# HKUST-Aerial-Robotics/DenseSurfelMapping

Measured on NVIDIA B200. Metric: frames/sec (KITTI 1226x370 depth+gray), higher is better.
Workload: dtype f32

## Files before the change

densesurfelmapping_b200/csrc/dsm_tile.cu:

```cuda
#include "dsm_exact.cuh"
#include <cuda_pipeline.h>

__device__ __forceinline__ unsigned smem_u32(const void *p) { return (unsigned)__cvta_generic_to_shared(p); }
__device__ __forceinline__ void mbar_init(unsigned bar, unsigned count)
{
    asm volatile("mbarrier.init.shared::cta.b64 [%0], %1;" ::"r"(bar), "r"(count) : "memory");
    asm volatile("fence.mbarrier_init.release.cluster;" ::: "memory");
}
__device__ __forceinline__ void mbar_expect_tx(unsigned bar, unsigned bytes)
{
    asm volatile("mbarrier.arrive.expect_tx.shared::cta.b64 _, [%0], %1;" ::"r"(bar), "r"(bytes) : "memory");
}
__device__ __forceinline__ void mbar_wait(unsigned bar, unsigned parity)
{
    unsigned ok = 0;
    for (unsigned spin = 0; !ok; spin++)
    {
        asm volatile("{\n\t.reg .pred p;\n\tmbarrier.try_wait.parity.shared::cta.b64 p, [%1], %2;\n\tselp.u32 %0, 1, 0, p;\n\t}"
                     : "=r"(ok)
                     : "r"(bar), "r"(parity)
                     : "memory");
        if (!ok && spin > (1u << 20)) __trap();
    }
}
__device__ __forceinline__ void tma_load_3d(unsigned dst, const CUtensorMap *map, int x, int y, int z, unsigned bar)
{
    asm volatile("cp.async.bulk.tensor.3d.shared::cluster.global.mbarrier::complete_tx::bytes [%0], [%1, {%3, %4, %5}], [%2];" ::"r"(dst),
                 "l"(reinterpret_cast<unsigned long long>(map)), "r"(bar), "r"(x), "r"(y), "r"(z)
                 : "memory");
}

#define A_EPS 3.814697265625e-06f
#define A_ALPHA 1e-10f
#define A_BIG 1e30f

__device__ __forceinline__ void relax_frame(const DsmDev &d, int b, int tid, int nthreads)
{
    const int n = __ldcg(&d.nlist[b]);
    if (n > 0)
    {
        const size_t fo = (size_t)b * d.px_stride;
        int2 *list = d.list + fo;
        int32_t *labels = d.labels + fo;
        uint8_t *codes = d.code + fo;
        int32_t *t = d.tstable + (size_t)b * d.S;
        for (;;)
        {
            int changed = 0;
            for (int e = tid; e < n; e += nthreads)
            {
                const int2 en = __ldcg(&list[e]);
                if (en.x < 0) continue;
                const int owner = __ldcg(&labels[en.x]);
                if (__ldcg(&t[owner]) < en.x)
                {
                    const int win = en.y & 0x0fffffff;
                    labels[en.x] = win;
                    codes[en.x] = (uint8_t)(en.y >> 28);
                    list[e].x = -1;
                    if (__ldcg(&t[win]) > en.x) atomicMin(&t[win], en.x);
                    changed = 1;
                }
            }
            if (!__syncthreads_or(changed)) break;
        }
    }
    if (tid == 0)
    {
        d.nlist[b] = 0;
        d.done[b] = 0;
    }
}

__device__ __forceinline__ float pick4(float a0, float a1, float a2, float a3, int i)
{
    return i == 0 ? a0 : (i == 1 ? a1 : (i == 2 ? a2 : a3));
}

#define DSM_CODE_NONE 4

template <bool FIRST>
__global__ void __launch_bounds__(128, 8) k_assign2(const __grid_constant__ DsmDev d)
{
    pdl_enter();
    __shared__ int s_last;
    const int b = d.frame0 + blockIdx.z;
    const int x4 = (blockIdx.x * 64 + threadIdx.x) * 4;
    const int y = blockIdx.y * blockDim.y + threadIdx.y;
    const int lane = threadIdx.x & 31;
    const bool active = (x4 < d.W) && (y < d.H);

    const size_t fo = (size_t)b * d.px_stride;
    const size_t so = (size_t)b * d.S;
    int wc[4] = {DSM_CODE_NONE, DSM_CODE_NONE, DSM_CODE_NONE, DSM_CODE_NONE};
    int oc[4] = {0, 0, 0, 0};
    int sidx0 = 0;
    if (active)
    {
        const size_t po = fo + (size_t)y * d.Wp + x4;
        const uchar4 g4 = *reinterpret_cast<const uchar4 *>(d.gray + po);
        float iv[4];
        if (FIRST)
        {
            const float4 z4 = *reinterpret_cast<const float4 *>(d.depth + po);
            iv[0] = (z4.x > F_0p01_LO) ? __frcp_rn(z4.x) : 0.0f;
            iv[1] = (z4.y > F_0p01_LO) ? __frcp_rn(z4.y) : 0.0f;
            iv[2] = (z4.z > F_0p01_LO) ? __frcp_rn(z4.z) : 0.0f;
            iv[3] = (z4.w > F_0p01_LO) ? __frcp_rn(z4.w) : 0.0f;
            *reinterpret_cast<float4 *>(d.invd + po) = make_float4(iv[0], iv[1], iv[2], iv[3]);
        }
        else
        {
            const float4 i4 = *reinterpret_cast<const float4 *>(d.invd + po);
            iv[0] = i4.x, iv[1] = i4.y, iv[2] = i4.z, iv[3] = i4.w;
            const uchar4 c4 = *reinterpret_cast<const uchar4 *>(d.code + po);
            oc[0] = c4.x, oc[1] = c4.y, oc[2] = c4.z, oc[3] = c4.w;
        }
        const float gi[4] = {(float)g4.x, (float)g4.y, (float)g4.z, (float)g4.w};
        const int bx = x4 >> 3, by = y >> 3, rx0 = x4 & 7, ry = y & 7;
        const int xa = (rx0 == 0) ? bx - 1 : bx, xb = xa + 1;
        const int ya = (ry < 4) ? by - 1 : by, yb = ya + 1;
        const bool vxa = xa >= 0 && xa < d.spw, vxb = xb >= 0 && xb < d.spw;
        const bool vya = ya >= 0 && ya < d.sph, vyb = (ry != 4) && yb >= 0 && yb < d.sph;
        sidx0 = ya * d.spw + xa;
        float sxq[4], sxq0[4], ayy[4], sI[4], shi[4], slo[4];
        bool sv[4];
        bool allmd = true, allmd0 = true;
        const float fyq = (float)y * 0.25f;
#pragma unroll
        for (int c = 0; c < 4; c++)
        {
            sv[c] = ((c >> 1) ? vxb : vxa) && ((c & 1) ? vyb : vya);
            const int li = sv[c] ? sidx0 + (c & 1) * d.spw + (c >> 1) : 0;
            const float4 s4 = d.seed[so + li];
            const float2 hl = d.seed_hl[so + li];
            sxq[c] = sv[c] ? s4.x * 0.25f : 1e18f;
            sxq0[c] = ((c >> 1) && rx0 == 4) ? 1e18f : sxq[c];
            const float ay = s4.y * 0.25f - fyq;
            ayy[c] = ay * ay;
            sI[c] = s4.z, shi[c] = hl.x, slo[c] = hl.y;
            const bool mdpos = s4.w > 0.f || !sv[c];
            allmd &= mdpos;
            if (!(c >> 1)) allmd0 &= mdpos;
        }
        if (rx0 != 4) allmd0 = allmd;
        unsigned uncertain = 0;
#pragma unroll
        for (int i = 0; i < 4; i++)
        {
            const float fxq = (float)(x4 + i) * 0.25f;
            const float pi = gi[i], pv = iv[i];
            const float w = (pv > 0.f && (i == 0 ? allmd0 : allmd)) ? 400.f : 0.f;
            float cost[4];
#pragma unroll
            for (int c = 0; c < 4; c++)
            {
                const float ax = (i == 0 ? sxq0[c] : sxq[c]) - fxq;
                const float n = fmaf(ax, ax, ayy[c]);
                const float idf = sI[c] - pi;
                const float cn = fmaf(idf * idf, 0.01f, n);
                const float t = (shi[c] - pv) + slo[c];
                cost[c] = fmaf(t * t, w, cn);
            }
            const float lo01 = fminf(cost[0], cost[1]), hi01 = fmaxf(cost[0], cost[1]);
            const float lo23 = fminf(cost[2], cost[3]), hi23 = fmaxf(cost[2], cost[3]);
            const float m1 = fminf(lo01, lo23);
            const float m2 = fminf(fminf(fmaxf(lo01, lo23), fminf(hi01, hi23)), A_BIG);
            wc[i] = cost[0] == m1 ? 0 : (cost[1] == m1 ? 1 : (cost[2] == m1 ? 2 : 3));
            const bool certain = (m2 - m1 > A_EPS * (m2 + m1) + A_ALPHA) && (m1 < 9e5f);
            if (!certain) uncertain |= 1u << i;
        }
        if (uncertain)
        {
            SeedC sc[4];
#pragma unroll
            for (int c = 0; c < 4; c++)
            {
                const int li = sv[c] ? sidx0 + (c & 1) * d.spw + (c >> 1) : 0;
                const float4 s4 = d.seed[so + li];
                sc[c].x = s4.x, sc[c].y = s4.y, sc[c].I = s4.z, sc[c].md = s4.w;
                sc[c].inv = d.inv_md[so + li];
            }
            const float fy = (float)y;
            while (uncertain)
            {
                const int i = __ffs(uncertain) - 1;
                uncertain &= uncertain - 1;
                const float fx = (float)(x4 + i);
                const float my_i = pick4(gi[0], gi[1], gi[2], gi[3], i);
                const float my_inv = pick4(iv[0], iv[1], iv[2], iv[3], i);
                const double my_inv_d = (double)my_inv;
                float min_d = 1e6f, min_nd = 1e6f;
                int idx_d = DSM_CODE_NONE, idx_nd = DSM_CODE_NONE;
                bool all_has_depth = true;
#pragma unroll
                for (int c = 0; c < 4; c++)
                {
                    const bool valid = sv[c] && ((c >> 1) ? !(rx0 == 4 && i == 0) : true);
                    float cnd, cdd;
                    const bool has = calc_cost(sc[c], my_i, my_inv, my_inv_d, fx, fy, cnd, cdd);
                    cdd = valid ? cdd : __int_as_float(0x7f800000);
                    cnd = valid ? cnd : __int_as_float(0x7f800000);
                    all_has_depth &= has || !valid;
                    const bool bd = cdd < min_d, bn = cnd < min_nd;
                    min_d = bd ? cdd : min_d;
                    idx_d = bd ? c : idx_d;
                    min_nd = bn ? cnd : min_nd;
                    idx_nd = bn ? c : idx_nd;
                }
                const int wv = all_has_depth ? idx_d : idx_nd;
                wc[0] = i == 0 ? wv : wc[0];
                wc[1] = i == 1 ? wv : wc[1];
                wc[2] = i == 2 ? wv : wc[2];
                wc[3] = i == 3 ? wv : wc[3];
            }
        }
#pragma unroll
        for (int i = 0; i < 4; i++)
            if (x4 + i >= d.W) wc[i] = DSM_CODE_NONE;
    }
    const int spw = d.spw;
    auto seed_of = [&](int c) { return c == DSM_CODE_NONE ? 0 : sidx0 + (c & 1) * spw + (c >> 1); };

    if (FIRST)
    {
        if (active)
        {
            const size_t po = fo + (size_t)y * d.Wp + x4;
            *reinterpret_cast<int4 *>(d.labels + po) = make_int4(seed_of(wc[0]), seed_of(wc[1]), seed_of(wc[2]), seed_of(wc[3]));
            *reinterpret_cast<uchar4 *>(d.code + po) = make_uchar4(wc[0], wc[1], wc[2], wc[3]);
        }
        return;
    }

    int2 ent[4];
    int nent = 0;
    if (active)
    {
        bool changed = false;
        const int32_t *ts = d.tstable + so;
#pragma unroll
        for (int i = 0; i < 4; i++)
        {
            if (x4 + i >= d.W || wc[i] == DSM_CODE_NONE || wc[i] == oc[i]) continue;
            const int pidx = y * d.Wp + x4 + i;
            const int win = seed_of(wc[i]);
            if (ts[seed_of(oc[i])] < 0)
            {
                oc[i] = wc[i];
                changed = true;
                if (ts[win] > pidx) atomicMin(&d.tstable[so + win], pidx);
            }
            else
            {
                ent[nent++] = make_int2(pidx, win | (wc[i] << 28));
            }
        }
        if (changed)
        {
            const size_t po = fo + (size_t)y * d.Wp + x4;
            *reinterpret_cast<int4 *>(d.labels + po) = make_int4(seed_of(oc[0]), seed_of(oc[1]), seed_of(oc[2]), seed_of(oc[3]));
            *reinterpret_cast<uchar4 *>(d.code + po) = make_uchar4(oc[0], oc[1], oc[2], oc[3]);
        }
    }
    if (__any_sync(FULL, nent > 0))
    {
        int total;
        const int excl = warp_excl_scan(nent, lane, total);
        int base = 0;
        if (lane == 31) base = atomicAdd(&d.nlist[b], total);
        base = __shfl_sync(FULL, base, 31);
        int2 *list = d.list + fo;
        for (int j = 0; j < nent; j++) list[base + excl + j] = ent[j];
    }
    const int tid = threadIdx.y * 64 + threadIdx.x;
    __syncthreads();
    if (tid == 0)
    {
        __threadfence();
        s_last = (atomicAdd(&d.done[b], 1) == (int)(gridDim.x * gridDim.y) - 1) ? 1 : 0;
    }
    __syncthreads();
    if (s_last)
    {
        __threadfence();
        relax_frame(d, b, tid, 128);
    }
}

#define DL_STRIDE 232
#define TILE_PLANE_BYTES 12544
#define TILE_BYTE_PLANE 4608
#define GAT_SMEM_DEP 0
#define GAT_SMEM_COD TILE_PLANE_BYTES
#define GAT_SMEM_GRY (TILE_PLANE_BYTES + TILE_BYTE_PLANE)
#define GAT_SMEM_LIST (TILE_PLANE_BYTES + 2 * TILE_BYTE_PLANE)
#define GAT_SMEM_ND (GAT_SMEM_LIST + 16 * DL_STRIDE * 4)
#define GAT_SMEM_BAR (GAT_SMEM_ND + 16 * 4)
#define GAT_SMEM_BYTES (GAT_SMEM_BAR + 16)
#define TILE_TX_BYTES (DSM_TILE_W * DSM_TILE_H * 4u + 2u * DSM_TILE_GW * DSM_TILE_H)

__device__ __forceinline__ unsigned zero_bytes_to_nibble(unsigned x)
{
    unsigned t = (x & 0x7f7f7f7fu) + 0x7f7f7f7fu;
    t = ~(t | x | 0x7f7f7f7fu);
    return ((t >> 7) * 0x00204081u >> 21) & 0xfu;
}
__device__ __forceinline__ unsigned member_mask16(const unsigned *codes, int r)
{
    const unsigned lo = (r < 8) ? 0x01010101u : 0u;
    const unsigned e_left = 0x02020202u | lo, e_right = lo;
    return zero_bytes_to_nibble(codes[0] ^ e_left) | (zero_bytes_to_nibble(codes[1] ^ e_left) << 4) |
           (zero_bytes_to_nibble(codes[2] ^ e_right) << 8) | (zero_bytes_to_nibble(codes[3] ^ e_right) << 12);
}

__device__ __forceinline__ int mask_index_sum(unsigned m)
{
    return __popc(m & 0xaaaau) + 2 * __popc(m & 0xccccu) + 4 * __popc(m & 0xf0f0u) + 8 * __popc(m & 0xff00u);
}
__device__ __forceinline__ unsigned nibble_to_bytes(unsigned n) { return (((n & 0xfu) * 0x00204081u) & 0x01010101u) * 0xffu; }

__global__ void __launch_bounds__(256, 6) k_gather(const __grid_constant__ DsmDev d, const __grid_constant__ DsmMaps mp)
{
    pdl_enter();
    extern __shared__ __align__(128) unsigned char smem[];
    const float *t_dep = reinterpret_cast<const float *>(smem + GAT_SMEM_DEP);
    const uint8_t *t_cod = smem + GAT_SMEM_COD, *t_gry = smem + GAT_SMEM_GRY;
    float *lists = reinterpret_cast<float *>(smem + GAT_SMEM_LIST);
    int *s_nd = reinterpret_cast<int *>(smem + GAT_SMEM_ND);
    const unsigned bar = smem_u32(smem + GAT_SMEM_BAR);

    const int b = d.frame0 + blockIdx.z;
    const int warp = threadIdx.x >> 5, lane = threadIdx.x & 31;
    const int X0 = blockIdx.x * (DSM_TILE_SX * DSM_SP) - DSM_SP / 2, Y0 = blockIdx.y * (DSM_TILE_SY * DSM_SP) - DSM_SP / 2;
    if (threadIdx.x == 0)
    {
        mbar_init(bar, 1);
        mbar_expect_tx(bar, TILE_TX_BYTES);
        tma_load_3d(smem_u32(smem + GAT_SMEM_DEP), &mp.dep, X0, Y0, b, bar);
        tma_load_3d(smem_u32(smem + GAT_SMEM_COD), &mp.cod, X0 - DSM_TILE_GX, Y0, b, bar);
        tma_load_3d(smem_u32(smem + GAT_SMEM_GRY), &mp.gry, X0 - DSM_TILE_GX, Y0, b, bar);
    }
    if (threadIdx.x == 1 && blockIdx.x == 0 && blockIdx.y == 0) d.nhard[b] = 0;
    const int W = d.W, H = d.H;
    const size_t so = (size_t)b * d.S;
    const int half = lane >> 4, r = lane & 15;
    int tflag[2];
#pragma unroll
    for (int rd = 0; rd < 2; rd++)
    {
        const int sl = rd * 16 + warp * 2 + half;
        const int sp_x = blockIdx.x * DSM_TILE_SX + (sl & 7), sp_y = blockIdx.y * DSM_TILE_SY + (sl >> 3);
        const bool live = sp_x < d.spw && sp_y < d.sph;
        tflag[rd] = live ? d.tstable[so + sp_y * d.spw + sp_x] : DSM_STABLE;
    }
    __syncthreads();
    mbar_wait(bar, 0);
#pragma unroll
    for (int rd = 0; rd < 2; rd++)
    {
        const int q = warp * 2 + half;
        const int sl = rd * 16 + q;
        const int tx = sl & 7, ty = sl >> 3;
        const int sp_x = blockIdx.x * DSM_TILE_SX + tx, sp_y = blockIdx.y * DSM_TILE_SY + ty;
        const int s = sp_y * d.spw + sp_x;
        const bool act = tflag[rd] != DSM_STABLE;
        const int x0 = sp_x * DSM_SP - DSM_SP / 2, y0 = sp_y * DSM_SP - DSM_SP / 2;
        const int xb = x0 > 0 ? x0 : 0, yb = y0 > 0 ? y0 : 0;
        const int xe = (x0 + 16) < W - 1 ? (x0 + 16) : W - 1;
        const int ye = (y0 + 16) < H - 1 ? (y0 + 16) : H - 1;
        const int y = y0 + r;
        const bool rowin = act && y >= yb && y < ye;
        const unsigned kmask = rowin ? (((1u << (xe - x0)) - 1u) & ~((1u << (xb - x0)) - 1u)) : 0u;
        const int trow = ty * DSM_SP + r, tcol = tx * DSM_SP;
        float zk[16];
        unsigned mm, zm = 0;
        {
            const unsigned *pc = reinterpret_cast<const unsigned *>(t_cod + trow * DSM_TILE_GW + DSM_TILE_GX + tcol);
            const unsigned cw[4] = {pc[0], pc[1], pc[2], pc[3]};
            mm = member_mask16(cw, r);
            const float4 *pz = reinterpret_cast<const float4 *>(t_dep + trow * DSM_TILE_W + tcol);
#pragma unroll
            for (int qd = 0; qd < 4; qd++)
            {
                const float4 z = pz[qd];
                zk[4 * qd] = z.x, zk[4 * qd + 1] = z.y, zk[4 * qd + 2] = z.z, zk[4 * qd + 3] = z.w;
            }
#pragma unroll
            for (int k = 0; k < 16; k++) zm |= (zk[k] > F_0p1_LO ? 1u : 0u) << k;
        }
        mm &= kmask;
        const unsigned dm = mm & zm;
        const int cnt = __popc(mm);
        const int sdx = mask_index_sum(mm);
        int si = 0;
        {
            const unsigned *pg = reinterpret_cast<const unsigned *>(t_gry + trow * DSM_TILE_GW + DSM_TILE_GX + tcol);
#pragma unroll
            for (int qd = 0; qd < 4; qd++) si = (int)__dp4a(pg[qd] & nibble_to_bytes(mm >> (4 * qd)), 0x01010101u, (unsigned)si);
        }
        int pa = cnt | (si << 8), pb = sdx | ((cnt * r) << 12);
#pragma unroll
        for (int o = 8; o > 0; o >>= 1)
        {
            pa += __shfl_xor_sync(FULL, pa, o);
            pb += __shfl_xor_sync(FULL, pb, o);
        }
        const int c = __popc(dm);
        int incl = c;
#pragma unroll
        for (int o = 1; o < 16; o <<= 1)
        {
            const int nb = __shfl_up_sync(FULL, incl, o, 16);
            if (r >= o) incl += nb;
        }
        const int ndt = __shfl_sync(FULL, incl, 15, 16);
        if (rd) __syncthreads();
        float *lp = lists + q * DL_STRIDE + (incl - c);
#pragma unroll
        for (int k = 0; k < 16; k++)
            if ((dm >> k) & 1u) *lp++ = zk[k];
        if (r == 0)
        {
            s_nd[q] = act ? ndt : 0;
            if (act)
            {
                const int n = pa & 0xff;
                d.usum[so + s] = make_int4(n, n * x0 + (pb & 0xfff), n * y0 + (pb >> 12), pa >> 8);
                d.und[so + s] = ndt;
            }
        }
        __syncthreads();
#pragma unroll
        for (int h2 = 0; h2 < 2; h2++)
        {
            const int q2 = warp + 8 * h2, n2 = s_nd[q2];
            if (n2 == 0) continue;
            const int sl2 = rd * 16 + q2;
            const int s2 = (blockIdx.y * DSM_TILE_SY + (sl2 >> 3)) * d.spw + blockIdx.x * DSM_TILE_SX + (sl2 & 7);
            float4 *dst = reinterpret_cast<float4 *>(d.dlist + (so + s2) * DL_STRIDE);
            const float4 *src = reinterpret_cast<const float4 *>(lists + q2 * DL_STRIDE);
            if (4 * lane < n2) dst[lane] = src[lane];
            if (4 * (lane + 32) < n2) dst[lane + 32] = src[lane + 32];
        }
    }
}

#define NW_T 64
#define NW_CAP 5632
__global__ void __launch_bounds__(NW_T, 8) k_newton2(const __grid_constant__ DsmDev d)
{
    pdl_enter();
    __shared__ __align__(16) float buf[NW_CAP];
    __shared__ int s_off[NW_T], s_wsum[NW_T / 32];
    const int b = d.frame0 + blockIdx.y;
    const int tid = threadIdx.x, lane = tid & 31, warp = tid >> 5;
    const int s = blockIdx.x * NW_T + tid;
    const size_t so = (size_t)b * d.S;
    const bool inr = s < d.S;
    const int tflag = inr ? d.tstable[so + s] : DSM_STABLE;
    const int nd_raw = inr ? d.und[so + s] : 0;
    const int4 su = inr ? d.usum[so + s] : make_int4(0, 0, 0, 0);
    const float4 pre = inr ? d.seed[so + s] : make_float4(0.f, 0.f, 0.f, 0.f);
    const bool act = tflag != DSM_STABLE;
    const int nd = act ? nd_raw : 0;
    {
        const int len4 = (nd + 3) & ~3;
        int wtot;
        const int wex = warp_excl_scan(len4, lane, wtot);
        if (lane == 31) s_wsum[warp] = wtot;
        __syncthreads();
        int base = 0;
        for (int w = 0; w < warp; w++) base += s_wsum[w];
// ... 393 lines not shown
        const int trow = p >> 7, tcol = p & 127;
        const float mz = t_dep[trow * DSM_TILE_W + tcol];
        const float ax = s_kx[tcol] * mz - mxs, ay = s_ky[trow] * mz - mys, az = mz - mzs;
        qx[j] = ax, qy[j] = ay, qz[j] = az;
        const float rr = ax * n0x + ay * n0y + az * n0z + 0.f;
        rnan |= !(rr == rr);
        margin = fminf(margin, fabsf(fabsf(rr) - d.huber_hi));
        qmax2 = fmaxf(qmax2, ax * ax + ay * ay + az * az);
        h[0] += (double)(2 * ax * ax), h[1] += (double)(2 * ax * ay), h[2] += (double)(2 * ax * az), h[3] += (double)(2 * ax);
        h[4] += (double)(2 * ay * ay), h[5] += (double)(2 * ay * az), h[6] += (double)(2 * ay);
        h[7] += (double)(2 * az * az), h[8] += (double)(2 * az);
        if (!(rr < d.huber_hi && rr > -d.huber_hi)) omask |= 1u << it;
    }
#pragma unroll
    for (int i = 0; i < 9; i++) h[i] = group8_sum_d(h[i]);
#pragma unroll
    for (int o = 4; o > 0; o >>= 1)
    {
        margin = fminf(margin, __shfl_xor_sync(FULL, margin, o));
        qmax2 = fmaxf(qmax2, __shfl_xor_sync(FULL, qmax2, o));
        rnan |= __shfl_xor_sync(FULL, rnan ? 1 : 0, o) != 0;
    }
    if (rnan) margin = __int_as_float(0x7fc00000);
    double *hr = d.hrec + (size_t)b * HREC * d.S + s;
    const size_t hs = (size_t)d.S;
    if (ok)
    {
#pragma unroll
        for (int i = 0; i < 9; i++)
            if ((i & 7) == gl) hr[i * hs] = h[i];
        if (gl == 7) hr[23 * hs] = __hiloint2double(__float_as_int(qmax2), __float_as_int(margin));
    }
    double ho[10] = {0, 0, 0, 0, 0, 0, 0, 0, 0, 0}, jo[4] = {0, 0, 0, 0};
    if (__any_sync(FULL, omask != 0))
    {
        while (omask)
        {
            const int it = __ffs(omask) - 1;
            omask &= omask - 1;
            const int p = pos[gl + 8 * it];
            const int trow = p >> 7, tcol = p & 127;
            const float mz = t_dep[trow * DSM_TILE_W + tcol];
            const float ax = s_kx[tcol] * mz - mxs, ay = s_ky[trow] * mz - mys, az = mz - mzs;
            const float rr = ax * n0x + ay * n0y + az * n0z + 0.f;
            ho[0] += (double)(2 * ax * ax), ho[1] += (double)(2 * ax * ay), ho[2] += (double)(2 * ax * az), ho[3] += (double)(2 * ax);
            ho[4] += (double)(2 * ay * ay), ho[5] += (double)(2 * ay * az), ho[6] += (double)(2 * ay);
            ho[7] += (double)(2 * az * az), ho[8] += (double)(2 * az), ho[9] += 2;
            if (rr >= d.huber_hi)
            {
                jo[0] += d.huber * (double)ax, jo[1] += d.huber * (double)ay, jo[2] += d.huber * (double)az, jo[3] += d.huber;
            }
            else if (rr <= -d.huber_hi)
            {
                jo[0] += -1 * d.huber * (double)ax, jo[1] += -1 * d.huber * (double)ay, jo[2] += -1 * d.huber * (double)az,
                    jo[3] += -1 * d.huber;
            }
        }
#pragma unroll
        for (int i = 0; i < 10; i++) ho[i] = group8_sum_d(ho[i]);
#pragma unroll
        for (int i = 0; i < 4; i++) jo[i] = group8_sum_d(jo[i]);
    }
    if (ok)
    {
        if (ho[9] != 0.0)
        {
#pragma unroll
            for (int i = 0; i < 14; i++)
                if ((i & 7) == gl) hr[(9 + i) * hs] = i < 10 ? ho[i] : jo[i - 10];
        }
        else if (gl == 0)
            hr[18 * hs] = 0.0;
    }
    if (live && gl == 0)
    {
        d.pfsum[(so + s) * 2] = ok ? make_float4(snx, sny, snz, maxd) : make_float4(0.f, 0.f, 0.f, maxd);
        d.pfsum[(so + s) * 2 + 1] = ok ? make_float4(mxs, mys, mzs, __int_as_float(ninl)) : make_float4(0.f, 0.f, 0.f, __int_as_float(0));
    }
}

__device__ __forceinline__ void solve4_spd_t(const double *h, double lambda, const double *j, double *u)
{
    const double a00 = h[0] + lambda, a01 = h[1], a02 = h[2], a03 = h[3];
    const double i0 = 1.0 / a00;
    const double l10 = a01 * i0, l20 = a02 * i0, l30 = a03 * i0;
    const double a11 = (h[4] + lambda) - l10 * a01, a12 = h[5] - l10 * a02, a13 = h[6] - l10 * a03;
    const double a22p = (h[7] + lambda) - l20 * a02, a23p = h[8] - l20 * a03, a33p = (h[9] + lambda) - l30 * a03;
    const double i1 = 1.0 / a11;
    const double l21 = a12 * i1, l31 = a13 * i1;
    const double a22 = a22p - l21 * a12, a23 = a23p - l21 * a13, a33q = a33p - l31 * a13;
    const double i2 = 1.0 / a22;
    const double l32 = a23 * i2;
    const double a33 = a33q - l32 * a23;
    const double y0 = j[0];
    const double y1 = j[1] - l10 * y0;
    const double y2 = j[2] - l20 * y0 - l21 * y1;
    const double y3 = j[3] - l30 * y0 - l31 * y1 - l32 * y2;
    u[3] = y3 / a33;
    u[2] = y2 * i2 - l32 * u[3];
    u[1] = y1 * i1 - l21 * u[2] - l31 * u[3];
    u[0] = y0 * i0 - l10 * u[1] - l20 * u[2] - l30 * u[3];
}

__device__ __forceinline__ void finish_plane(const DsmDev &d, size_t o, const float4 &sd, const float4 &P0, const float4 &P1, float nx, float ny,
                                             float nz, float nb)
{
    nb = nb - (nx * P1.x + ny * P1.y + nz * P1.z);
    const float nl = sqrtf(nx * nx + ny * ny + nz * nz);
    nx /= nl;
    ny /= nl;
    nz /= nl;
    nb /= nl;
    const float axf = (sd.x - d.cx) / d.fx * sd.w;
    const float ayf = (sd.y - d.cy) / d.fy * sd.w;
    double ax = (double)axf, ay = (double)ayf, az = (double)sd.w;
    const float kk = (float)(-1 * (ax * (double)nx + ay * (double)ny + az * (double)nz) - (double)nb);
    ax += (double)(kk * nx);
    ay += (double)(kk * ny);
    az += (double)(kk * nz);
    const float mean_depth = (float)az;
    float view_cos = (float)(-1.0 * ((double)nx * ax + (double)ny * ay + (double)nz * az) / sqrt(ax * ax + ay * ay + az * az));
    if (view_cos < 0)
    {
        view_cos = -view_cos;
        nx = -nx;
        ny = -ny;
        nz = -nz;
    }
    float4 *pl = d.plane + o * 3;
    pl[0] = make_float4(nx, ny, nz, view_cos);
    pl[1] = make_float4((float)ax, (float)ay, (float)az, mean_depth);
    pl[2] = make_float4(sqrtf(P0.w), sd.z, sd.x, sd.y);
}

__device__ __forceinline__ float gn_step(const double *hh0, const double *jo, float qmax, float &nx, float &ny, float &nz, float &nb)
{
    double jj[4];
    const double tx = (double)nx, ty = (double)ny, tz = (double)nz, tb = (double)nb;
    jj[0] = ((hh0[0] * tx + hh0[1] * ty) + hh0[2] * tz) + hh0[3] * tb + jo[0];
    jj[1] = ((hh0[1] * tx + hh0[4] * ty) + hh0[5] * tz) + hh0[6] * tb + jo[1];
    jj[2] = ((hh0[2] * tx + hh0[5] * ty) + hh0[7] * tz) + hh0[8] * tb + jo[2];
    jj[3] = ((hh0[3] * tx + hh0[6] * ty) + hh0[8] * tz) + hh0[9] * tb + jo[3];
    double u[4];
    solve4_spd_t(hh0, 5.0, jj, u);
    const float ox = nx, oy = ny, oz = nz, ob = nb;
    nx = (float)((double)nx - u[0]);
    ny = (float)((double)ny - u[1]);
    nz = (float)((double)nz - u[2]);
    nb = (float)((double)nb - u[3]);
    const float dx = nx - ox, dy = ny - oy, dz = nz - oz;
    return qmax * sqrtf(dx * dx + dy * dy + dz * dz) * 1.0001f + fabsf(nb - ob) + 1e-4f;
}

#define GS_CAP 9216
__global__ void __launch_bounds__(128, 4) k_gn_solve(const __grid_constant__ DsmDev d)
{
    pdl_enter();
    __shared__ __align__(16) float pts[GS_CAP];
    __shared__ float4 s_theta[128];
    __shared__ int s_queue[128], s_gn[128], s_poff[128], s_nq, s_used;
    const int b = d.frame0 + blockIdx.y;
    const int tid = threadIdx.x, lane = tid & 31, warp = tid >> 5;
    const int s = blockIdx.x * 128 + tid;
    const size_t so = (size_t)b * d.S;
    const size_t hs = (size_t)d.S;
    if (tid == 0) s_nq = 0, s_used = 0;
    __syncthreads();
    if (s < d.S)
    {
        const float4 sd = d.seed[so + s];
        const float4 P0 = d.pfsum[(so + s) * 2], P1 = d.pfsum[(so + s) * 2 + 1];
        const int n = __float_as_int(P1.w);
        if (n <= 0)
        {
            float4 *pl = d.plane + (so + s) * 3;
            pl[0] = make_float4(0.f, 0.f, 0.f, 0.f);
            pl[1] = make_float4(0.f, 0.f, 0.f, sd.w);
            pl[2] = make_float4(0.f, sd.z, sd.x, sd.y);
        }
        else
        {
            const float len0 = sqrtf(P0.x * P0.x + P0.y * P0.y + P0.z * P0.z);
            float nx = P0.x / len0, ny = P0.y / len0, nz = P0.z / len0, nb = 0.f;
            const double *hr = d.hrec + (size_t)b * HREC * d.S + s;
            double hh0[10], jo[4] = {0, 0, 0, 0};
#pragma unroll
            for (int i = 0; i < 9; i++) hh0[i] = hr[i * hs];
            hh0[9] = 2.0 * (double)n;
            if (hr[18 * hs] != 0.0)
            {
#pragma unroll
                for (int i = 0; i < 10; i++) hh0[i] -= hr[(9 + i) * hs];
#pragma unroll
                for (int i = 0; i < 4; i++) jo[i] = hr[(19 + i) * hs];
            }
            const double pk = hr[23 * hs];
            const float margin = __int_as_float(__double2loint(pk));
            const float qmax = sqrtf(__int_as_float(__double2hiint(pk)));
            float moved = 0.f;
            int gn = 0;
            for (; gn < 5; gn++)
            {
                if (gn > 0 && !(moved + 2e-3f < margin)) break;
                moved += gn_step(hh0, jo, qmax, nx, ny, nz, nb);
            }
            if (gn == 5)
                finish_plane(d, so + s, sd, P0, P1, nx, ny, nz, nb);
            else
            {
                const int q = atomicAdd(&s_nq, 1);
                const int len4 = (n + 3) & ~3;
                const int off = atomicAdd(&s_used, 3 * len4);
                s_queue[q] = tid;
                s_gn[tid] = gn;
                s_poff[tid] = (off + 3 * len4 <= GS_CAP) ? off : -1;
                s_theta[tid] = make_float4(nx, ny, nz, nb);
            }
        }
    }
    __syncthreads();
    const int nq = s_nq;
    if (nq == 0) return;
    for (int q = warp; q < nq; q += 4)
    {
        const int t2 = s_queue[q], off = s_poff[t2];
        if (off < 0) continue;
        const size_t o2 = so + blockIdx.x * 128 + t2;
        const int n2 = __float_as_int(d.pfsum[o2 * 2 + 1].w), l4 = ((n2 + 3) & ~3) >> 2;
        const float4 *src = reinterpret_cast<const float4 *>(d.qlist + o2 * (3 * PL_STRIDE));
        float4 *dst = reinterpret_cast<float4 *>(pts + off);
        for (int pln = 0; pln < 3; pln++)
            for (int j4 = lane; j4 < l4; j4 += 32) __pipeline_memcpy_async(dst + pln * l4 + j4, src + pln * (PL_STRIDE / 4) + j4, 16);
    }
    __pipeline_commit();
    __pipeline_wait_prior(0);
    __syncthreads();
    for (int q = tid; q < nq; q += 128)
    {
        const int t2 = s_queue[q];
        const size_t o2 = so + blockIdx.x * 128 + t2;
        const float4 sd = d.seed[o2];
        const float4 P0 = d.pfsum[o2 * 2], P1 = d.pfsum[o2 * 2 + 1];
        const int n = __float_as_int(P1.w), l4 = ((n + 3) & ~3) >> 2;
        const double *hr = d.hrec + (size_t)b * HREC * d.S + (blockIdx.x * 128 + t2);
        const float qmax = sqrtf(__int_as_float(__double2hiint(hr[23 * hs])));
        const float4 th = s_theta[t2];
        float nx = th.x, ny = th.y, nz = th.z, nb = th.w;
        const int off = s_poff[t2];
        const float4 *qx = off >= 0 ? reinterpret_cast<const float4 *>(pts + off) : reinterpret_cast<const float4 *>(d.qlist + o2 * (3 * PL_STRIDE));
        const int pstride = off >= 0 ? l4 : PL_STRIDE / 4;
        float margin = 0.f, moved = 0.f;
        double hh0[10], jo[4];
        for (int gn = s_gn[t2]; gn < 5; gn++)
        {
            if (!(moved + 2e-3f < margin))
            {
#pragma unroll
                for (int i = 0; i < 9; i++) hh0[i] = hr[i * hs];
                hh0[9] = 2.0 * (double)n;
#pragma unroll
                for (int i = 0; i < 4; i++) jo[i] = 0.0;
                float mg = __int_as_float(0x7f800000);
                bool rnan = false;
                auto point = [&](float ax, float ay, float az)
                {
                    const float r = ax * nx + ay * ny + az * nz + nb;
                    rnan |= !(r == r);
                    mg = fminf(mg, fabsf(fabsf(r) - d.huber_hi));
                    if (!(r < d.huber_hi && r > -d.huber_hi))
                    {
                        hh0[0] -= (double)(2 * ax * ax), hh0[1] -= (double)(2 * ax * ay), hh0[2] -= (double)(2 * ax * az), hh0[3] -= (double)(2 * ax);
                        hh0[4] -= (double)(2 * ay * ay), hh0[5] -= (double)(2 * ay * az), hh0[6] -= (double)(2 * ay);
                        hh0[7] -= (double)(2 * az * az), hh0[8] -= (double)(2 * az), hh0[9] -= 2;
                        if (r >= d.huber_hi)
                        {
                            jo[0] += d.huber * (double)ax, jo[1] += d.huber * (double)ay;
                            jo[2] += d.huber * (double)az, jo[3] += d.huber;
                        }
                        else if (r <= -d.huber_hi)
                        {
                            jo[0] += -1 * d.huber * (double)ax, jo[1] += -1 * d.huber * (double)ay;
                            jo[2] += -1 * d.huber * (double)az, jo[3] += -1 * d.huber;
                        }
                    }
                };
                int k = 0;
                for (; k + 4 <= n; k += 4)
                {
                    const float4 a = qx[k >> 2], bb = qx[pstride + (k >> 2)], c = qx[2 * pstride + (k >> 2)];
                    point(a.x, bb.x, c.x);
                    point(a.y, bb.y, c.y);
                    point(a.z, bb.z, c.z);
                    point(a.w, bb.w, c.w);
                }
                if (k < n)
                {
                    const float4 a = qx[k >> 2], bb = qx[pstride + (k >> 2)], c = qx[2 * pstride + (k >> 2)];
                    point(a.x, bb.x, c.x);
                    if (k + 1 < n) point(a.y, bb.y, c.y);
                    if (k + 2 < n) point(a.z, bb.z, c.z);
                }
                margin = rnan ? __int_as_float(0x7fc00000) : mg;
                moved = 0.f;
            }
            moved += gn_step(hh0, jo, qmax, nx, ny, nz, nb);
        }
        finish_plane(d, o2, sd, P0, P1, nx, ny, nz, nb);
    }
}

int dsm_tile_setup()
{
    cudaError_t e = cudaFuncSetAttribute(k_gather, cudaFuncAttributeMaxDynamicSharedMemorySize, GAT_SMEM_BYTES);
    if (e == cudaSuccess) e = cudaFuncSetAttribute(k_plane_gather, cudaFuncAttributeMaxDynamicSharedMemorySize, PG_SMEM_BYTES);
    if (e == cudaSuccess) e = cudaFuncSetAttribute(k_gather, cudaFuncAttributePreferredSharedMemoryCarveout, 100);
    if (e == cudaSuccess) e = cudaFuncSetAttribute(k_plane_gather, cudaFuncAttributePreferredSharedMemoryCarveout, 100);
    return e == cudaSuccess ? 0 : -1;
}
void dsm_launch_assign2(const DsmDev &d, int nb, bool first, cudaStream_t s)
{
    dim3 block(64, 2);
    dim3 grid((d.W + 255) / 256, (d.H + 1) / 2, nb);
    if (first)
        pdl_launch(k_assign2<true>, grid, block, 0, s, d);
    else
        pdl_launch(k_assign2<false>, grid, block, 0, s, d);
}
void dsm_launch_gather(const DsmDev &d, const DsmMaps &m, int nb, cudaStream_t s)
{
    dim3 grid((d.spw + DSM_TILE_SX - 1) / DSM_TILE_SX, (d.sph + DSM_TILE_SY - 1) / DSM_TILE_SY, nb);
    pdl_launch(k_gather, grid, dim3(256), GAT_SMEM_BYTES, s, d, m);
}
void dsm_launch_newton2(const DsmDev &d, int nb, cudaStream_t s)
{
    dim3 grid((d.S + NW_T - 1) / NW_T, nb);
    pdl_launch(k_newton2, grid, dim3(NW_T), 0, s, d);
    pdl_launch(k_newton_hard, grid, dim3(NW_T), 0, s, d);
}
void dsm_launch_plane_gather(const DsmDev &d, const DsmMaps &m, int nb, cudaStream_t s)
{
    dim3 grid((d.spw + DSM_TILE_SX - 1) / DSM_TILE_SX, (d.sph + DSM_TILE_SY - 1) / DSM_TILE_SY, nb);
    pdl_launch(k_plane_gather, grid, dim3(256), PG_SMEM_BYTES, s, d, m);
}
void dsm_launch_gn_solve(const DsmDev &d, int nb, cudaStream_t s)
{
    dim3 grid((d.S + 127) / 128, nb);
    pdl_launch(k_gn_solve, grid, dim3(128), 0, s, d);
}
```

Baseline: 37470.

## Split Gauss-Newton point accumulation across 8 lanes per surfel with shuffle reduction

The Gauss-Newton solve previously ran one thread per queued surfel and looped serially over all of that surfel's points. Now a group of 8 lanes shares each surfel: each lane accumulates a strided subset of points into local Hessian and gradient partials, and the partials are combined with xor shuffles before the solve. This targets long serial loops and poor occupancy when only a few surfels are queued. In exchange it changes the double-precision summation order, makes all 8 lanes repeat the redundant 4x4 solve, and adds warp-wide synchronisation that can force idle lanes to wait.

```diff
diff --git a/densesurfelmapping_b200/csrc/dsm_tile.cu b/densesurfelmapping_b200/csrc/dsm_tile.cu
--- a/densesurfelmapping_b200/csrc/dsm_tile.cu
+++ b/densesurfelmapping_b200/csrc/dsm_tile.cu
@@ -1018,6 +1018,7 @@
     return qmax * sqrtf(dx * dx + dy * dy + dz * dz) * 1.0001f + fabsf(nb - ob) + 1e-4f;
 }
 
+#define GN_LANES 8
 #define GS_CAP 9216
 __global__ void __launch_bounds__(128, 4) k_gn_solve(const __grid_constant__ DsmDev d)
 {
@@ -1101,77 +1102,83 @@
     __pipeline_commit();
     __pipeline_wait_prior(0);
     __syncthreads();
-    for (int q = tid; q < nq; q += 128)
-    {
-        const int t2 = s_queue[q];
+    const int gq = tid / GN_LANES, gl = tid % GN_LANES;
+    for (int q0 = 0; q0 < nq; q0 += 128 / GN_LANES)
+    {
+        const int q = q0 + gq;
+        if (!__any_sync(FULL, q < nq)) break;
+        const bool has = q < nq;
+        const int t2 = has ? s_queue[q] : 0;
         const size_t o2 = so + blockIdx.x * 128 + t2;
-        const float4 sd = d.seed[o2];
-        const float4 P0 = d.pfsum[o2 * 2], P1 = d.pfsum[o2 * 2 + 1];
-        const int n = __float_as_int(P1.w), l4 = ((n + 3) & ~3) >> 2;
+        const float4 P1 = has ? d.pfsum[o2 * 2 + 1] : make_float4(0.f, 0.f, 0.f, 0.f);
+        const int n = has ? __float_as_int(P1.w) : 0, l4 = ((n + 3) & ~3) >> 2;
         const double *hr = d.hrec + (size_t)b * HREC * d.S + (blockIdx.x * 128 + t2);
-        const float qmax = sqrtf(__int_as_float(__double2hiint(hr[23 * hs])));
-        const float4 th = s_theta[t2];
+        const float qmax = has ? sqrtf(__int_as_float(__double2hiint(hr[23 * hs]))) : 0.f;
+        const float4 th = has ? s_theta[t2] : make_float4(0.f, 0.f, 0.f, 0.f);
         float nx = th.x, ny = th.y, nz = th.z, nb = th.w;
-        const int off = s_poff[t2];
-        const float4 *qx = off >= 0 ? reinterpret_cast<const float4 *>(pts + off) : reinterpret_cast<const float4 *>(d.qlist + o2 * (3 * PL_STRIDE));
-        const int pstride = off >= 0 ? l4 : PL_STRIDE / 4;
+        const int off = has ? s_poff[t2] : 0;
+        const float *qx = off >= 0 ? pts + off : d.qlist + o2 * (3 * PL_STRIDE);
+        const int pstride = off >= 0 ? 4 * l4 : PL_STRIDE;
+        const int g0 = has ? s_gn[t2] : 5;
         float margin = 0.f, moved = 0.f;
         double hh0[10], jo[4];
-        for (int gn = s_gn[t2]; gn < 5; gn++)
-        {
-            if (!(moved + 2e-3f < margin))
-            {
-#pragma unroll
-                for (int i = 0; i < 9; i++) hh0[i] = hr[i * hs];
-                hh0[9] = 2.0 * (double)n;
-#pragma unroll
-                for (int i = 0; i < 4; i++) jo[i] = 0.0;
+        for (int gn = 0; gn < 5; gn++)
+        {
+            const bool act = gn >= g0;
+            const bool cls = act && !(moved + 2e-3f < margin);
+            if (__any_sync(FULL, cls))
+            {
+                double ho[10] = {0, 0, 0, 0, 0, 0, 0, 0, 0, 0}, rj[4] = {0, 0, 0, 0};
                 float mg = __int_as_float(0x7f800000);
                 bool rnan = false;
-                auto point = [&](float ax, float ay, float az)
+                const int nc = cls ? n : 0;
+                for (int k = gl; k < nc; k += GN_LANES)
                 {
+                    const float ax = qx[k], ay = qx[pstride + k], az = qx[2 * pstride + k];
                     const float r = ax * nx + ay * ny + az * nz + nb;
                     rnan |= !(r == r);
                     mg = fminf(mg, fabsf(fabsf(r) - d.huber_hi));
                     if (!(r < d.huber_hi && r > -d.huber_hi))
                     {
-                        hh0[0] -= (double)(2 * ax * ax), hh0[1] -= (double)(2 * ax * ay), hh0[2] -= (double)(2 * ax * az), hh0[3] -= (double)(2 * ax);
-                        hh0[4] -= (double)(2 * ay * ay), hh0[5] -= (double)(2 * ay * az), hh0[6] -= (double)(2 * ay);
-                        hh0[7] -= (double)(2 * az * az), hh0[8] -= (double)(2 * az), hh0[9] -= 2;
+                        ho[0] += (double)(2 * ax * ax), ho[1] += (double)(2 * ax * ay), ho[2] += (double)(2 * ax * az), ho[3] += (double)(2 * ax);
+                        ho[4] += (double)(2 * ay * ay), ho[5] += (double)(2 * ay * az), ho[6] += (double)(2 * ay);
+                        ho[7] += (double)(2 * az * az), ho[8] += (double)(2 * az), ho[9] += 2;
                         if (r >= d.huber_hi)
                         {
-                            jo[0] += d.huber * (double)ax, jo[1] += d.huber * (double)ay;
-                            jo[2] += d.huber * (double)az, jo[3] += d.huber;
+                            rj[0] += d.huber * (double)ax, rj[1] += d.huber * (double)ay;
+                            rj[2] += d.huber * (double)az, rj[3] += d.huber;
                         }
                         else if (r <= -d.huber_hi)
                         {
-                            jo[0] += -1 * d.huber * (double)ax, jo[1] += -1 * d.huber * (double)ay;
-                            jo[2] += -1 * d.huber * (double)az, jo[3] += -1 * d.huber;
+                            rj[0] += -1 * d.huber * (double)ax, rj[1] += -1 * d.huber * (double)ay;
+                            rj[2] += -1 * d.huber * (double)az, rj[3] += -1 * d.huber;
                         }
                     }
-                };
-                int k = 0;
-                for (; k + 4 <= n; k += 4)
+                }
+#pragma unroll
+                for (int o = GN_LANES / 2; o > 0; o >>= 1)
                 {
-                    const float4 a = qx[k >> 2], bb = qx[pstride + (k >> 2)], c = qx[2 * pstride + (k >> 2)];
-                    point(a.x, bb.x, c.x);
-                    point(a.y, bb.y, c.y);
-                    point(a.z, bb.z, c.z);
-                    point(a.w, bb.w, c.w);
+#pragma unroll
+                    for (int i = 0; i < 10; i++) ho[i] += __shfl_xor_sync(FULL, ho[i], o);
+#pragma unroll
+                    for (int i = 0; i < 4; i++) rj[i] += __shfl_xor_sync(FULL, rj[i], o);
+                    mg = fminf(mg, __shfl_xor_sync(FULL, mg, o));
+                    rnan |= __shfl_xor_sync(FULL, rnan ? 1 : 0, o) != 0;
                 }
-                if (k < n)
+                if (cls)
                 {
-                    const float4 a = qx[k >> 2], bb = qx[pstride + (k >> 2)], c = qx[2 * pstride + (k >> 2)];
-                    point(a.x, bb.x, c.x);
-                    if (k + 1 < n) point(a.y, bb.y, c.y);
-                    if (k + 2 < n) point(a.z, bb.z, c.z);
+#pragma unroll
+                    for (int i = 0; i < 9; i++) hh0[i] = hr[i * hs] - ho[i];
+                    hh0[9] = 2.0 * (double)n - ho[9];
+#pragma unroll
+                    for (int i = 0; i < 4; i++) jo[i] = rj[i];
+                    margin = rnan ? __int_as_float(0x7fc00000) : mg;
+                    moved = 0.f;
                 }
-                margin = rnan ? __int_as_float(0x7fc00000) : mg;
-                moved = 0.f;
-            }
-            moved += gn_step(hh0, jo, qmax, nx, ny, nz, nb);
-        }
-        finish_plane(d, o2, sd, P0, P1, nx, ny, nz, nb);
+            }
+            if (act) moved += gn_step(hh0, jo, qmax, nx, ny, nz, nb);
+        }
+        if (has && gl == 0) finish_plane(d, o2, d.seed[o2], d.pfsum[o2 * 2], P1, nx, ny, nz, nb);
     }
 }
 
```

Result: no change. 37640, median of 6 (+0.5%).

## Retile assign kernel around seed cells with shared-memory seed staging

Applied to the files above, without the earlier changes.

Restructures k_assign2 so each thread handles an 8-pixel run aligned to seed-cell boundaries and each block covers a 16x8 seed-aligned tile. The seed data for the block's two seed rows is staged once into shared memory instead of every thread loading four seeds from global memory. Per-pixel winner codes are packed into byte words, and change detection uses SIMD byte compares. In exchange it adds a __syncthreads, more registers per thread, and uncertain pixels now reload gray and depth from global memory.

```diff
diff --git a/densesurfelmapping_b200/csrc/dsm_tile.cu b/densesurfelmapping_b200/csrc/dsm_tile.cu
--- a/densesurfelmapping_b200/csrc/dsm_tile.cu
+++ b/densesurfelmapping_b200/csrc/dsm_tile.cu
@@ -30,9 +30,19 @@
                  : "memory");
 }
 
+__device__ __forceinline__ unsigned zero_bytes_to_nibble(unsigned x)
+{
+    unsigned t = (x & 0x7f7f7f7fu) + 0x7f7f7f7fu;
+    t = ~(t | x | 0x7f7f7f7fu);
+    return ((t >> 7) * 0x00204081u >> 21) & 0xfu;
+}
+__device__ __forceinline__ unsigned nibble_to_bytes(unsigned n) { return (((n & 0xfu) * 0x00204081u) & 0x01010101u) * 0xffu; }
+
 #define A_EPS 3.814697265625e-06f
 #define A_ALPHA 1e-10f
 #define A_BIG 1e30f
+#define ASG_TX 16
+#define ASG_COLS (ASG_TX + 1)
 
 __device__ __forceinline__ void relax_frame(const DsmDev &d, int b, int tid, int nthreads)
 {
@@ -72,90 +82,119 @@
     }
 }
 
-__device__ __forceinline__ float pick4(float a0, float a1, float a2, float a3, int i)
-{
-    return i == 0 ? a0 : (i == 1 ? a1 : (i == 2 ? a2 : a3));
-}
-
 #define DSM_CODE_NONE 4
+#define DSM_CODE_NONE4 0x04040404u
+
+__device__ __forceinline__ int seed_of_code(unsigned c, int sidx0, int spw)
+{
+    return c == DSM_CODE_NONE ? 0 : sidx0 + (int)(c & 1u) * spw + (int)(c >> 1);
+}
+__device__ __forceinline__ int4 labels_of_codes(unsigned w, int sidx0, int spw)
+{
+    return make_int4(seed_of_code(w & 0xffu, sidx0, spw), seed_of_code((w >> 8) & 0xffu, sidx0, spw),
+                     seed_of_code((w >> 16) & 0xffu, sidx0, spw), seed_of_code(w >> 24, sidx0, spw));
+}
+__device__ __forceinline__ float inv_depth(float z) { return z > F_0p01_LO ? __frcp_rn(z) : 0.0f; }
 
 template <bool FIRST>
 __global__ void __launch_bounds__(128, 8) k_assign2(const __grid_constant__ DsmDev d)
 {
     pdl_enter();
+    __shared__ float4 s_sd[2][ASG_COLS];
+    __shared__ float s_syq[2][ASG_COLS];
+    __shared__ int s_md[ASG_COLS];
     __shared__ int s_last;
     const int b = d.frame0 + blockIdx.z;
-    const int x4 = (blockIdx.x * 64 + threadIdx.x) * 4;
-    const int y = blockIdx.y * blockDim.y + threadIdx.y;
-    const int lane = threadIdx.x & 31;
-    const bool active = (x4 < d.W) && (y < d.H);
-
-    const size_t fo = (size_t)b * d.px_stride;
-    const size_t so = (size_t)b * d.S;
-    int wc[4] = {DSM_CODE_NONE, DSM_CODE_NONE, DSM_CODE_NONE, DSM_CODE_NONE};
-    int oc[4] = {0, 0, 0, 0};
-    int sidx0 = 0;
-    if (active)
-    {
-        const size_t po = fo + (size_t)y * d.Wp + x4;
-        const uchar4 g4 = *reinterpret_cast<const uchar4 *>(d.gray + po);
-        float iv[4];
-        if (FIRST)
-        {
-            const float4 z4 = *reinterpret_cast<const float4 *>(d.depth + po);
-            iv[0] = (z4.x > F_0p01_LO) ? __frcp_rn(z4.x) : 0.0f;
-            iv[1] = (z4.y > F_0p01_LO) ? __frcp_rn(z4.y) : 0.0f;
-            iv[2] = (z4.z > F_0p01_LO) ? __frcp_rn(z4.z) : 0.0f;
-            iv[3] = (z4.w > F_0p01_LO) ? __frcp_rn(z4.w) : 0.0f;
-            *reinterpret_cast<float4 *>(d.invd + po) = make_float4(iv[0], iv[1], iv[2], iv[3]);
-        }
-        else
-        {
-            const float4 i4 = *reinterpret_cast<const float4 *>(d.invd + po);
-            iv[0] = i4.x, iv[1] = i4.y, iv[2] = i4.z, iv[3] = i4.w;
-            const uchar4 c4 = *reinterpret_cast<const uchar4 *>(d.code + po);
-            oc[0] = c4.x, oc[1] = c4.y, oc[2] = c4.z, oc[3] = c4.w;
-        }
-        const float gi[4] = {(float)g4.x, (float)g4.y, (float)g4.z, (float)g4.w};
-        const int bx = x4 >> 3, by = y >> 3, rx0 = x4 & 7, ry = y & 7;
-        const int xa = (rx0 == 0) ? bx - 1 : bx, xb = xa + 1;
-        const int ya = (ry < 4) ? by - 1 : by, yb = ya + 1;
-        const bool vxa = xa >= 0 && xa < d.spw, vxb = xb >= 0 && xb < d.spw;
-        const bool vya = ya >= 0 && ya < d.sph, vyb = (ry != 4) && yb >= 0 && yb < d.sph;
-        sidx0 = ya * d.spw + xa;
-        float sxq[4], sxq0[4], ayy[4], sI[4], shi[4], slo[4];
-        bool sv[4];
-        bool allmd = true, allmd0 = true;
-        const float fyq = (float)y * 0.25f;
-#pragma unroll
-        for (int c = 0; c < 4; c++)
-        {
-            sv[c] = ((c >> 1) ? vxb : vxa) && ((c & 1) ? vyb : vya);
-            const int li = sv[c] ? sidx0 + (c & 1) * d.spw + (c >> 1) : 0;
+    const int tx = threadIdx.x, ty = threadIdx.y, tid = ty * ASG_TX + tx, lane = tid & 31;
+    const int ya = (int)blockIdx.y - 1;
+    const int y = 8 * ya + 4 + ty;
+    const int xa = ASG_TX * (int)blockIdx.x - 1 + tx;
+    const int x0 = 8 * xa + 4;
+    const bool row0 = ty == 0;
+    const int spw = d.spw;
+    const int sidx0 = ya * spw + xa;
+    const size_t so = (size_t)b * d.S, fo = (size_t)b * d.px_stride;
+    const int po = y * d.Wp + x0;
+    const int nx = min(d.W - x0, 8);
+    const unsigned pm = (y >= 0 && y < d.H && nx > 0) ? ((1u << nx) - 1u) & (xa < 0 ? 0xf0u : 0xffu) : 0u;
+
+    unsigned gw[2] = {0u, 0u}, ocw[2] = {0u, 0u};
+    float iv[8];
+#pragma unroll
+    for (int q = 0; q < 2; q++)
+    {
+        const bool ld = (pm >> (4 * q)) & 1u;
+        const int o = po + 4 * q;
+        float4 v = make_float4(0.f, 0.f, 0.f, 0.f);
+        if (ld)
+        {
+            gw[q] = *reinterpret_cast<const unsigned *>(d.gray + fo + o);
+            if (FIRST)
+            {
+                v = *reinterpret_cast<const float4 *>(d.depth + fo + o);
+                v = make_float4(inv_depth(v.x), inv_depth(v.y), inv_depth(v.z), inv_depth(v.w));
+                *reinterpret_cast<float4 *>(d.invd + fo + o) = v;
+            }
+            else
+            {
+                v = *reinterpret_cast<const float4 *>(d.invd + fo + o);
+                ocw[q] = *reinterpret_cast<const unsigned *>(d.code + fo + o);
+            }
+        }
+        iv[4 * q] = v.x, iv[4 * q + 1] = v.y, iv[4 * q + 2] = v.z, iv[4 * q + 3] = v.w;
+    }
+
+    if (tid < ASG_COLS)
+    {
+        const int j = xa - tx + tid;
+        int md = 0;
+#pragma unroll
+        for (int r = 0; r < 2; r++)
+        {
+            const int sr = ya + r;
+            const bool v = j >= 0 && j < spw && sr >= 0 && sr < d.sph;
+            const int li = v ? sr * spw + j : 0;
             const float4 s4 = d.seed[so + li];
             const float2 hl = d.seed_hl[so + li];
-            sxq[c] = sv[c] ? s4.x * 0.25f : 1e18f;
-            sxq0[c] = ((c >> 1) && rx0 == 4) ? 1e18f : sxq[c];
-            const float ay = s4.y * 0.25f - fyq;
+            s_sd[r][tid] = make_float4(v ? s4.x * 0.25f : 1e18f, s4.z, hl.x, hl.y);
+            s_syq[r][tid] = s4.y * 0.25f;
+            md |= (s4.w > 0.f || !v) ? 1 << r : 0;
+        }
+        s_md[tid] = md;
+    }
+    __syncthreads();
+
+    unsigned wcw[2] = {DSM_CODE_NONE4, DSM_CODE_NONE4};
+    if (pm)
+    {
+        const float4 c0 = s_sd[0][tx], c1 = s_sd[1][tx], c2 = s_sd[0][tx + 1], c3 = s_sd[1][tx + 1];
+        const float sxq[4] = {c0.x, row0 ? 1e18f : c1.x, c2.x, row0 ? 1e18f : c3.x};
+        const float sI[4] = {c0.y, c1.y, c2.y, c3.y}, shi[4] = {c0.z, c1.z, c2.z, c3.z}, slo[4] = {c0.w, c1.w, c2.w, c3.w};
+        const float syq[4] = {s_syq[0][tx], s_syq[1][tx], s_syq[0][tx + 1], s_syq[1][tx + 1]};
+        const float fyq = (float)y * 0.25f;
+        float ayy[4];
+#pragma unroll
+        for (int c = 0; c < 4; c++)
+        {
+            const float ay = syq[c] - fyq;
             ayy[c] = ay * ay;
-            sI[c] = s4.z, shi[c] = hl.x, slo[c] = hl.y;
-            const bool mdpos = s4.w > 0.f || !sv[c];
-            allmd &= mdpos;
-            if (!(c >> 1)) allmd0 &= mdpos;
-        }
-        if (rx0 != 4) allmd0 = allmd;
-        unsigned uncertain = 0;
-#pragma unroll
-        for (int i = 0; i < 4; i++)
-        {
-            const float fxq = (float)(x4 + i) * 0.25f;
-            const float pi = gi[i], pv = iv[i];
+        }
+        const int mrow = row0 ? 2 : 0;
+        const int mda = s_md[tx] | mrow, mdb = s_md[tx + 1] | mrow;
+        const bool allmd = (mda & mdb) == 3, allmd0 = mda == 3;
+        const float fxq0 = (float)x0 * 0.25f;
+        unsigned wlo = 0u, whi = 0u, uncertain = 0u;
+#pragma unroll
+        for (int i = 0; i < 8; i++)
+        {
+            const float fxq = i == 0 ? fxq0 : fxq0 + 0.25f * (float)i;
+            const float pi = (float)((gw[i >> 2] >> (8 * (i & 3))) & 0xffu), pv = iv[i];
             const float w = (pv > 0.f && (i == 0 ? allmd0 : allmd)) ? 400.f : 0.f;
             float cost[4];
 #pragma unroll
             for (int c = 0; c < 4; c++)
             {
-                const float ax = (i == 0 ? sxq0[c] : sxq[c]) - fxq;
+                const float ax = ((i == 0 && (c >> 1)) ? 1e18f : sxq[c]) - fxq;
                 const float n = fmaf(ax, ax, ayy[c]);
                 const float idf = sI[c] - pi;
                 const float cn = fmaf(idf * idf, 0.01f, n);
@@ -166,17 +205,23 @@
             const float lo23 = fminf(cost[2], cost[3]), hi23 = fmaxf(cost[2], cost[3]);
             const float m1 = fminf(lo01, lo23);
             const float m2 = fminf(fminf(fmaxf(lo01, lo23), fminf(hi01, hi23)), A_BIG);
-            wc[i] = cost[0] == m1 ? 0 : (cost[1] == m1 ? 1 : (cost[2] == m1 ? 2 : 3));
+            const unsigned wc = (lo23 == m1 ? 2u : 0u) | ((cost[1] == m1 || cost[3] == m1) ? 1u : 0u);
+            if (i < 4) wlo |= wc << (8 * i);
+            else whi |= wc << (8 * (i - 4));
             const bool certain = (m2 - m1 > A_EPS * (m2 + m1) + A_ALPHA) && (m1 < 9e5f);
             if (!certain) uncertain |= 1u << i;
         }
+        uncertain &= pm;
         if (uncertain)
         {
             SeedC sc[4];
+            bool sv[4];
 #pragma unroll
             for (int c = 0; c < 4; c++)
             {
-                const int li = sv[c] ? sidx0 + (c & 1) * d.spw + (c >> 1) : 0;
+                const int sx = xa + (c >> 1), sy = ya + (c & 1);
+                sv[c] = sx >= 0 && sx < spw && sy >= 0 && sy < d.sph && !(row0 && (c & 1));
+                const int li = sv[c] ? sy * spw + sx : 0;
                 const float4 s4 = d.seed[so + li];
                 sc[c].x = s4.x, sc[c].y = s4.y, sc[c].I = s4.z, sc[c].md = s4.w;
                 sc[c].inv = d.inv_md[so + li];
@@ -186,9 +231,9 @@
             {
                 const int i = __ffs(uncertain) - 1;
                 uncertain &= uncertain - 1;
-                const float fx = (float)(x4 + i);
-                const float my_i = pick4(gi[0], gi[1], gi[2], gi[3], i);
-                const float my_inv = pick4(iv[0], iv[1], iv[2], iv[3], i);
+                const float fx = (float)(x0 + i);
+                const float my_i = (float)d.gray[fo + po + i];
+                const float my_inv = FIRST ? inv_depth(d.depth[fo + po + i]) : d.invd[fo + po + i];
                 const double my_inv_d = (double)my_inv;
                 float min_d = 1e6f, min_nd = 1e6f;
                 int idx_d = DSM_CODE_NONE, idx_nd = DSM_CODE_NONE;
@@ -196,7 +241,7 @@
 #pragma unroll
                 for (int c = 0; c < 4; c++)
                 {
-                    const bool valid = sv[c] && ((c >> 1) ? !(rx0 == 4 && i == 0) : true);
+                    const bool valid = sv[c] && !((c >> 1) && i == 0);
                     float cnd, cdd;
                     const bool has = calc_cost(sc[c], my_i, my_inv, my_inv_d, fx, fy, cnd, cdd);
                     cdd = valid ? cdd : __int_as_float(0x7f800000);
@@ -208,61 +253,62 @@
                     min_nd = bn ? cnd : min_nd;
                     idx_nd = bn ? c : idx_nd;
                 }
-                const int wv = all_has_depth ? idx_d : idx_nd;
-                wc[0] = i == 0 ? wv : wc[0];
-                wc[1] = i == 1 ? wv : wc[1];
-                wc[2] = i == 2 ? wv : wc[2];
-                wc[3] = i == 3 ? wv : wc[3];
-            }
-        }
-#pragma unroll
-        for (int i = 0; i < 4; i++)
-            if (x4 + i >= d.W) wc[i] = DSM_CODE_NONE;
-    }
-    const int spw = d.spw;
-    auto seed_of = [&](int c) { return c == DSM_CODE_NONE ? 0 : sidx0 + (c & 1) * spw + (c >> 1); };
+                const unsigned wv = (unsigned)(all_has_depth ? idx_d : idx_nd);
+                const int sh = 8 * (i & 3);
+                if (i < 4) wlo = (wlo & ~(0xffu << sh)) | (wv << sh);
+                else whi = (whi & ~(0xffu << sh)) | (wv << sh);
+            }
+        }
+        const unsigned bm0 = nibble_to_bytes(pm), bm1 = nibble_to_bytes(pm >> 4);
+        wcw[0] = (wlo & bm0) | (DSM_CODE_NONE4 & ~bm0);
+        wcw[1] = (whi & bm1) | (DSM_CODE_NONE4 & ~bm1);
+    }
 
     if (FIRST)
     {
-        if (active)
-        {
-            const size_t po = fo + (size_t)y * d.Wp + x4;
-            *reinterpret_cast<int4 *>(d.labels + po) = make_int4(seed_of(wc[0]), seed_of(wc[1]), seed_of(wc[2]), seed_of(wc[3]));
-            *reinterpret_cast<uchar4 *>(d.code + po) = make_uchar4(wc[0], wc[1], wc[2], wc[3]);
-        }
+#pragma unroll
+        for (int q = 0; q < 2; q++)
+            if ((pm >> (4 * q)) & 1u)
+            {
+                *reinterpret_cast<int4 *>(d.labels + fo + po + 4 * q) = labels_of_codes(wcw[q], sidx0, spw);
+                *reinterpret_cast<unsigned *>(d.code + fo + po + 4 * q) = wcw[q];
+            }
         return;
     }
 
-    int2 ent[4];
-    int nent = 0;
-    if (active)
-    {
-        bool changed = false;
+    unsigned sw = zero_bytes_to_nibble(~(__vcmpne4(wcw[0], ocw[0]) & __vcmpne4(wcw[0], DSM_CODE_NONE4))) |
+                  (zero_bytes_to_nibble(~(__vcmpne4(wcw[1], ocw[1]) & __vcmpne4(wcw[1], DSM_CODE_NONE4))) << 4);
+    const unsigned long long wc64 = wcw[0] | ((unsigned long long)wcw[1] << 32);
+    unsigned deferred = 0;
+    if (sw)
+    {
         const int32_t *ts = d.tstable + so;
-#pragma unroll
-        for (int i = 0; i < 4; i++)
-        {
-            if (x4 + i >= d.W || wc[i] == DSM_CODE_NONE || wc[i] == oc[i]) continue;
-            const int pidx = y * d.Wp + x4 + i;
-            const int win = seed_of(wc[i]);
-            if (ts[seed_of(oc[i])] < 0)
-            {
-                oc[i] = wc[i];
-                changed = true;
-                if (ts[win] > pidx) atomicMin(&d.tstable[so + win], pidx);
+        const unsigned long long oc64 = ocw[0] | ((unsigned long long)ocw[1] << 32);
+        unsigned long long cm = 0;
+        while (sw)
+        {
+            const int i = __ffs(sw) - 1;
+            sw &= sw - 1;
+            const int win = seed_of_code((unsigned)(wc64 >> (8 * i)) & 0xffu, sidx0, spw);
+            if (ts[seed_of_code((unsigned)(oc64 >> (8 * i)) & 0xffu, sidx0, spw)] < 0)
+            {
+                cm |= 0xffull << (8 * i);
+                if (ts[win] > po + i) atomicMin(&d.tstable[so + win], po + i);
             }
             else
-            {
-                ent[nent++] = make_int2(pidx, win | (wc[i] << 28));
-            }
-        }
-        if (changed)
-        {
-            const size_t po = fo + (size_t)y * d.Wp + x4;
-            *reinterpret_cast<int4 *>(d.labels + po) = make_int4(seed_of(oc[0]), seed_of(oc[1]), seed_of(oc[2]), seed_of(oc[3]));
-            *reinterpret_cast<uchar4 *>(d.code + po) = make_uchar4(oc[0], oc[1], oc[2], oc[3]);
-        }
-    }
+                deferred |= 1u << i;
+        }
+        const unsigned long long nc = (oc64 & ~cm) | (wc64 & cm);
+#pragma unroll
+        for (int q = 0; q < 2; q++)
+            if ((unsigned)(cm >> (32 * q)))
+            {
+                const unsigned w = (unsigned)(nc >> (32 * q));
+                *reinterpret_cast<int4 *>(d.labels + fo + po + 4 * q) = labels_of_codes(w, sidx0, spw);
+                *reinterpret_cast<unsigned *>(d.code + fo + po + 4 * q) = w;
+            }
+    }
+    const int nent = __popc(deferred);
     if (__any_sync(FULL, nent > 0))
     {
         int total;
@@ -270,10 +316,15 @@
         int base = 0;
         if (lane == 31) base = atomicAdd(&d.nlist[b], total);
         base = __shfl_sync(FULL, base, 31);
-        int2 *list = d.list + fo;
-        for (int j = 0; j < nent; j++) list[base + excl + j] = ent[j];
-    }
-    const int tid = threadIdx.y * 64 + threadIdx.x;
+        int2 *list = d.list + fo + base + excl;
+        while (deferred)
+        {
+            const int i = __ffs(deferred) - 1;
+            deferred &= deferred - 1;
+            const unsigned c = (unsigned)(wc64 >> (8 * i)) & 0xffu;
+            *list++ = make_int2(po + i, seed_of_code(c, sidx0, spw) | (int)(c << 28));
+        }
+    }
     __syncthreads();
     if (tid == 0)
     {
@@ -284,7 +335,7 @@
     if (s_last)
     {
         __threadfence();
-        relax_frame(d, b, tid, 128);
+        relax_frame(d, b, tid, ASG_TX * 8);
     }
 }
 
@@ -300,12 +351,6 @@
 #define GAT_SMEM_BYTES (GAT_SMEM_BAR + 16)
 #define TILE_TX_BYTES (DSM_TILE_W * DSM_TILE_H * 4u + 2u * DSM_TILE_GW * DSM_TILE_H)
 
-__device__ __forceinline__ unsigned zero_bytes_to_nibble(unsigned x)
-{
-    unsigned t = (x & 0x7f7f7f7fu) + 0x7f7f7f7fu;
-    t = ~(t | x | 0x7f7f7f7fu);
-    return ((t >> 7) * 0x00204081u >> 21) & 0xfu;
-}
 __device__ __forceinline__ unsigned member_mask16(const unsigned *codes, int r)
 {
     const unsigned lo = (r < 8) ? 0x01010101u : 0u;
@@ -318,7 +363,6 @@
 {
     return __popc(m & 0xaaaau) + 2 * __popc(m & 0xccccu) + 4 * __popc(m & 0xf0f0u) + 8 * __popc(m & 0xff00u);
 }
-__device__ __forceinline__ unsigned nibble_to_bytes(unsigned n) { return (((n & 0xfu) * 0x00204081u) & 0x01010101u) * 0xffu; }
 
 __global__ void __launch_bounds__(256, 6) k_gather(const __grid_constant__ DsmDev d, const __grid_constant__ DsmMaps mp)
 {
@@ -1185,8 +1229,8 @@
 }
 void dsm_launch_assign2(const DsmDev &d, int nb, bool first, cudaStream_t s)
 {
-    dim3 block(64, 2);
-    dim3 grid((d.W + 255) / 256, (d.H + 1) / 2, nb);
+    dim3 block(ASG_TX, 8);
+    dim3 grid((d.W + 4 + 8 * ASG_TX - 1) / (8 * ASG_TX), (d.H + 4 + 7) / 8, nb);
     if (first)
         pdl_launch(k_assign2<true>, grid, block, 0, s, d);
     else
```

Result: faster. 37440 before, 41930 after (median of 6 runs) (+12.0%).
